# fakerlove1/HPFG

Hardware: AMD Instinct MI355X
Metric: labeled+unlabeled images/sec/node, U-Net 224x224 ACDC-shaped (Mean-Teacher step) (higher is better)
Workload: dtype bf16x3 (fp32 storage; products as split-bf16 MFMA hi*hi+hi*lo+lo*hi, fp32 accumulate); 1 GPU; mean_teacher_unet_224x224 (BASELINE configs[1]): U-Net 1ch->4cls, 8 labelled + 8 unlabelled per GPU, student fwd+bwd + train-mode teacher fwd + CE/Dice/MSE + SGD + EMA; size=224, hipgraph=True, sync_bn=False, parallelism=dp1, math=bf16x3

## Files before the change

### hpfg_amd/csrc/wgrad.hip

```cpp
#include <cstdlib>
#include "wgrad_kernel.h"
#include "wgrad_bf16_kernel.h"

namespace {

__global__ __launch_bounds__(256) void slab_reduce_kernel(const float* __restrict__ slab, float* __restrict__ dw, int S, int taps, int Cin,
                                                          int CinPad, int Cout, int CoutPad) {
  __shared__ float red[16][17];
  const long per = (long)taps * CinPad * CoutPad;
  const int il = threadIdx.x & 15, sl = threadIdx.x >> 4;
  const long i = (long)blockIdx.x * 16 + il;
  float t0 = 0.f, t1 = 0.f;
  if (i < per) {
    int s = sl;
    for (; s + 16 < S; s += 32) {
      t0 += slab[s * per + i];
      t1 += slab[(s + 16) * per + i];
    }
    if (s < S) t0 += slab[s * per + i];
  }
  red[sl][il] = t0 + t1;
  __syncthreads();
  if (sl == 0 && i < per) {
    float t = 0.f;
#pragma unroll
    for (int k = 0; k < 16; ++k) t += red[k][il];
    int co = (int)(i % CoutPad);
    int ci = (int)((i / CoutPad) % CinPad);
    int tap = (int)(i / ((long)CoutPad * CinPad));
    if (co < Cout && ci < Cin) dw[((long)co * Cin + ci) * taps + tap] = t;
  }
}

__global__ __launch_bounds__(256) void slab_reduce_multi_kernel(const HpfgSlabDesc* __restrict__ table) {
  __shared__ float red[16][65];
  const HpfgSlabDesc d = table[blockIdx.y];
  const long per = (long)d.taps * d.CinPad * d.CoutPad;
  const int il = threadIdx.x & 15, sl = threadIdx.x >> 4;
  const bool vec = (per & 3) == 0;
  for (long g0 = (long)blockIdx.x * 64; g0 < per; g0 += (long)gridDim.x * 64) {
    const long i = g0 + il * 4;
    f32x4 t0 = {0.f, 0.f, 0.f, 0.f}, t1 = t0;
    if (vec && i + 3 < per) {
      int s = sl;
      f32x4 t2 = t0, t3 = t0;
      for (; s + 48 < d.S; s += 64) {
        t0 += *reinterpret_cast<const f32x4*>(d.slab + s * per + i);
        t1 += *reinterpret_cast<const f32x4*>(d.slab + (s + 16) * per + i);
        t2 += *reinterpret_cast<const f32x4*>(d.slab + (s + 32) * per + i);
        t3 += *reinterpret_cast<const f32x4*>(d.slab + (s + 48) * per + i);
      }
      for (; s < d.S; s += 16) t0 += *reinterpret_cast<const f32x4*>(d.slab + s * per + i);
      t0 += t2;
      t1 += t3;
    } else {
      for (int s = sl; s < d.S; s += 16)
#pragma unroll
        for (int j = 0; j < 4; ++j)
          if (i + j < per) t0[j] += d.slab[s * per + i + j];
    }
    __syncthreads();
#pragma unroll
    for (int j = 0; j < 4; ++j) red[sl][il * 4 + j] = t0[j] + t1[j];
    __syncthreads();
    if (threadIdx.x < 64) {
      const long e = g0 + threadIdx.x;
      if (e < per) {
        float t = 0.f;
#pragma unroll
        for (int k = 0; k < 16; ++k) t += red[k][threadIdx.x];
        const int co = (int)(e % d.CoutPad), ci = (int)((e / d.CoutPad) % d.CinPad), tap = (int)(e / ((long)d.CoutPad * d.CinPad));
        if (co < d.Cout && ci < d.Cin) d.dw_oihw[((long)co * d.Cin + ci) * d.taps + tap] = t;
      }
    }
  }
}

__global__ __launch_bounds__(256) void channel_sum_stage1(const float* __restrict__ g, int pstride, long npix, int C, float* __restrict__ scratch) {
  __shared__ float red[256 * 4];
  const int tid = threadIdx.x;
  if ((C & 3) == 0 && (pstride & 3) == 0) {
    const int Q = C >> 2, q = tid % Q, pl = tid / Q, PL = 256 / Q;
    f32x4 a = {0.f, 0.f, 0.f, 0.f};
    if (pl < PL) {
      const long stride = (long)gridDim.x * PL;
      for (long pix = (long)blockIdx.x * PL + pl; pix < npix; pix += 4 * stride) {
#pragma unroll
        for (int u = 0; u < 4; ++u) {
          const long px = pix + u * stride;
          if (px < npix) a += *reinterpret_cast<const f32x4*>(g + px * pstride + q * 4);
        }
      }
    }
#pragma unroll
    for (int j = 0; j < 4; ++j) red[tid * 4 + j] = a[j];
    __syncthreads();
    if (tid < C) {
      float t = 0.f;
      const int qq = tid >> 2, j = tid & 3;
      for (int l = 0; l < PL; ++l) t += red[(l * Q + qq) * 4 + j];
      scratch[(long)blockIdx.x * C + tid] = t;
    }
    return;
  }
  const int c = tid % C, pl = tid / C, PL = 256 / C;
  float a = 0.f;
  if (pl < PL)
    for (long pix = (long)blockIdx.x * PL + pl; pix < npix; pix += (long)gridDim.x * PL) a += g[pix * pstride + c];
  red[tid] = a;
  __syncthreads();
  if (tid < C) {
    float t = 0.f;
    for (int l = 0; l < PL; ++l) t += red[l * C + tid];
    scratch[(long)blockIdx.x * C + tid] = t;
  }
}

__global__ __launch_bounds__(64) void channel_sum_stage2(const float* __restrict__ scratch, int nblk, int C, float* __restrict__ out) {
  const int c = blockIdx.x;
  double a = 0.0;
  for (int i = threadIdx.x; i < nblk; i += 64) a += (double)scratch[(long)i * C + c];
#pragma unroll
  for (int o = 32; o >= 1; o >>= 1) a += __shfl_xor(a, o);
  if (threadIdx.x == 0) out[c] = (float)a;
}

}

extern "C" int hpfg_wgrad_splits(int N, int H, int W, int CinPad, int CoutPad, int taps) {
  (void)taps;
  using namespace hpfg_wg;
  int ni, nj;
  hpfg_wg16::pick_shape(CinPad, CoutPad, &ni, &nj);
  long pairs = (long)(CinPad / (16 * ni)) * (CoutPad / (16 * nj));
  long nwork = (long)N * ((H + TH - 1) / TH) * ((W + TW - 1) / TW);
  const long resident = 512;
  long target = resident / pairs;
  if (target < 1) target = 1;
  if (target > nwork) target = nwork;
  long per_block = (nwork + target - 1) / target;
  return (int)((nwork + per_block - 1) / per_block);
}

extern "C" long hpfg_wgrad_slab_floats(int N, int H, int W, int CinPad, int CoutPad, int taps) {
  return (long)hpfg_wgrad_splits(N, H, W, CinPad, CoutPad, taps) * taps * CinPad * CoutPad;
}

extern "C" int hpfg_wgrad(const HpfgWgradArgs* a, void* stream) {
  HPFG_ARG_CHECK(a && a->slab && a->dw_oihw, "wgrad: null pointer");
  HPFG_ARG_CHECK(a->taps == 9 || a->taps == 1, "wgrad: taps must be 1 or 9");
  HPFG_ARG_CHECK(a->CinPad % 16 == 0 && a->CoutPad % 16 == 0 && a->Cin <= a->CinPad && a->Cout <= a->CoutPad, "wgrad: bad channel padding");
  HPFG_ARG_CHECK(a->S >= 1, "wgrad: S < 1");
  HPFG_ARG_CHECK(a->a1.mode == HPFG_ACT_NONE || a->a0.C % 16 == 0, "wgrad: concat needs a0.C %% 16 == 0");
  hipStream_t st = (hipStream_t)stream;
  const int akind = hpfg_kind_of(a->a0, a->a1);
  HPFG_ARG_CHECK(akind >= 0 && akind != HPFG_KIND_DZ, "wgrad: unsupported input source (a0.mode=%d, a1.mode=%d)", a->a0.mode, a->a1.mode);
  int rc = 1;
  const bool b16 = (a->math & 0xff) == HPFG_MATH_BF16X3 && a->taps == 9;
  if ((a->math & 0xff) == HPFG_MATH_BF16X3 && a->taps == 1 && (a->g.mode == HPFG_ACT_PLAIN || a->g.mode == HPFG_ACT_STRIDED) && a->g.C % 4 == 0)
    rc = hpfg_wgrad16_launch_1x1(*a, akind, st);
  if (a->g.mode == HPFG_ACT_SPLIT16 || akind == HPFG_KIND_SPLIT) {
    HPFG_ARG_CHECK(b16, "wgrad: SPLIT16 sources are a feature of the 3x3 bf16x3 kernel");
    rc = hpfg_wgrad16_launch_split(*a, akind, st);
  } else if (rc != 1) {
  } else if (b16 && a->g.mode == HPFG_ACT_DZ) rc = hpfg_wgrad16_launch_dz(*a, akind, st);
  else if (b16 && (a->g.mode == HPFG_ACT_PLAIN || a->g.mode == HPFG_ACT_STRIDED)) rc = hpfg_wgrad16_launch_plain(*a, akind, st);
  else if (a->g.mode == HPFG_ACT_DZ) rc = hpfg_wgrad_launch_dz(*a, akind, st);
  else if (a->g.mode == HPFG_ACT_PLAIN || a->g.mode == HPFG_ACT_STRIDED) rc = hpfg_wgrad_launch_plain(*a, akind, st);
  else {
    hpfg_set_error("wgrad: unsupported gradient source mode %d", a->g.mode);
    return -1;
  }
  if (rc || a->defer_reduce) return rc;
  long per = (long)a->taps * a->CinPad * a->CoutPad;
  hipLaunchKernelGGL(slab_reduce_kernel, dim3((unsigned)((per + 15) / 16)), dim3(256), 0, st, a->slab, a->dw_oihw, a->S, a->taps, a->Cin, a->CinPad,
                     a->Cout, a->CoutPad);
  return hpfg_launch_status("slab_reduce_kernel");
}

extern "C" int hpfg_slab_reduce_multi(const HpfgSlabDesc* table_dev, const HpfgSlabDesc* table_host, int nlayers, void* stream) {
  HPFG_ARG_CHECK(table_dev && table_host && nlayers > 0 && nlayers < 65536, "slab_reduce_multi: bad args");
  long mx = 0;
  for (int i = 0; i < nlayers; ++i) {
    long per = (long)table_host[i].taps * table_host[i].CinPad * table_host[i].CoutPad;
    if (per > mx) mx = per;
  }
  long gx = (mx + 63) / 64;
  if (gx > 2048) gx = 2048;
  hipLaunchKernelGGL(slab_reduce_multi_kernel, dim3((unsigned)gx, nlayers), dim3(256), 0, (hipStream_t)stream, table_dev);
  return hpfg_launch_status("slab_reduce_multi_kernel");
}

extern "C" int hpfg_channel_sum_blocks(long npix, int C) {
  if (C < 1 || C > 256 || npix < 1) return 0;
  const int PL = 256 / C;
  const long want = (npix + PL - 1) / PL;
  return (int)(want < 512 ? want : 512);
}

extern "C" int hpfg_channel_sum_partials(const float* g, int pstride, long npix, int C, float* partials, void* stream) {
  HPFG_ARG_CHECK(g && partials && C >= 1 && C <= 256 && npix > 0, "channel_sum_partials: bad args");
  hipLaunchKernelGGL(channel_sum_stage1, dim3(hpfg_channel_sum_blocks(npix, C)), dim3(256), 0, (hipStream_t)stream, g, pstride, npix, C, partials);
  return hpfg_launch_status("channel_sum_stage1");
}

extern "C" int hpfg_channel_sum(const float* g, int pstride, long npix, int C, float* out, float* scratch, void* stream) {
  HPFG_ARG_CHECK(g && out && scratch && C >= 1 && C <= 256 && npix > 0, "channel_sum: bad args");
  int PL = 256 / C;
  long want = (npix + PL - 1) / PL;
  int nblk = (int)(want < 512 ? want : 512);
  hipLaunchKernelGGL(channel_sum_stage1, dim3(nblk), dim3(256), 0, (hipStream_t)stream, g, pstride, npix, C, scratch);
  hipLaunchKernelGGL(channel_sum_stage2, dim3(C), dim3(64), 0, (hipStream_t)stream, scratch, nblk, C, out);
  return hpfg_launch_status("channel_sum");
}
```

Baseline: 7877 images/s.

## Rewrite multi-layer slab reduction with per-layer geometry plans and flattened grid

Replaces the 2D-grid slab reduction, where every layer got the same number of blocks sized by the largest layer, with a flattened 1D grid. A host-computed plan gives each layer exactly the blocks it needs. Each layer picks one of four strategies from its shape: a few-slab quad path that transposes through LDS for coalesced OIHW writes, lane and part paths with deep batched loads for many slabs, or a scalar row fallback. The aim is to remove idle blocks, increase memory-level parallelism and improve write coalescing, at the cost of much more complex code and a per-block linear search for its layer.

```diff
diff --git a/hpfg_amd/csrc/wgrad.hip b/hpfg_amd/csrc/wgrad.hip
--- a/hpfg_amd/csrc/wgrad.hip
+++ b/hpfg_amd/csrc/wgrad.hip
@@ -32,47 +32,269 @@
   }
 }
 
-__global__ __launch_bounds__(256) void slab_reduce_multi_kernel(const HpfgSlabDesc* __restrict__ table) {
-  __shared__ float red[16][65];
-  const HpfgSlabDesc d = table[blockIdx.y];
+constexpr int SR_THREADS = 256;
+constexpr int SR_MAX_LAYERS = 32;
+constexpr int SR_LDS_FLOATS = 1152;
+enum { SR_QUAD = 0, SR_LANES = 1, SR_PARTS = 2, SR_ROWS = 3 };
+
+struct SrGeom {
+  int kind, CW, R, ncb, nrb;
+};
+struct SrPlan {
+  int n;
+  int start[SR_MAX_LAYERS + 1];
+};
+
+__host__ __device__ HPFG_NO_PK_F32 inline SrGeom sr_geom(const HpfgSlabDesc& d) {
+  SrGeom g;
   const long per = (long)d.taps * d.CinPad * d.CoutPad;
-  const int il = threadIdx.x & 15, sl = threadIdx.x >> 4;
-  const bool vec = (per & 3) == 0;
-  for (long g0 = (long)blockIdx.x * 64; g0 < per; g0 += (long)gridDim.x * 64) {
-    const long i = g0 + il * 4;
-    f32x4 t0 = {0.f, 0.f, 0.f, 0.f}, t1 = t0;
-    if (vec && i + 3 < per) {
-      int s = sl;
-      f32x4 t2 = t0, t3 = t0;
-      for (; s + 48 < d.S; s += 64) {
-        t0 += *reinterpret_cast<const f32x4*>(d.slab + s * per + i);
-        t1 += *reinterpret_cast<const f32x4*>(d.slab + (s + 16) * per + i);
-        t2 += *reinterpret_cast<const f32x4*>(d.slab + (s + 32) * per + i);
-        t3 += *reinterpret_cast<const f32x4*>(d.slab + (s + 48) * per + i);
+  g.CW = g.R = 0, g.nrb = 1;
+  if (d.CinPad % 16 || d.CoutPad % 16 || ((uintptr_t)d.slab & 15)) {
+    g.kind = SR_ROWS, g.ncb = (int)((per + 15) / 16);
+  } else if (d.S <= 16) {
+    g.kind = SR_QUAD;
+    g.CW = d.CoutPad % 32 == 0 ? 32 : 16;
+    g.R = SR_THREADS / (d.taps * (g.CW / 4));
+    g.ncb = (d.Cout + g.CW - 1) / g.CW;
+    g.nrb = (d.Cin + g.R - 1) / g.R;
+  } else {
+    const int nq = d.taps * d.Cin * ((d.Cout + 3) / 4);
+    g.kind = d.S > 256 && per < (1L << 23) ? SR_PARTS : SR_LANES;
+    g.ncb = g.kind == SR_PARTS ? (nq + 3) / 4 : (nq + 15) / 16;
+  }
+  return g;
+}
+
+__device__ __forceinline__ HPFG_NO_PK_F32 void sr_barrier() {
+  __builtin_amdgcn_fence(__ATOMIC_RELEASE, "workgroup");
+  __builtin_amdgcn_s_barrier();
+  __builtin_amdgcn_fence(__ATOMIC_ACQUIRE, "workgroup");
+}
+
+#define SR_GLOBAL __attribute__((address_space(1)))
+template <typename T>
+__device__ __forceinline__ HPFG_NO_PK_F32 T sr_ld(const float* row, unsigned vbyte) {
+  return *(const SR_GLOBAL T*)((const SR_GLOBAL char*)row + vbyte);
+}
+
+template <typename T, int B>
+__device__ __forceinline__ HPFG_NO_PK_F32 void sr_batch(const float*& row, long rs, unsigned vbyte, T& t0, T& t1, T& t2, T& t3) {
+  T x[B];
+#pragma unroll
+  for (int i = 0; i < B; ++i) x[i] = sr_ld<T>(row + i * rs, vbyte);
+#pragma unroll
+  for (int i = 0; i < B; i += 4) {
+    t0 += x[i];
+    t1 += x[i + 1];
+    t2 += x[i + 2];
+    t3 += x[i + 3];
+  }
+  row += B * rs;
+}
+
+template <typename T>
+__device__ __forceinline__ HPFG_NO_PK_F32 T sr_chain(const float* row, long rs, unsigned vbyte, int nfull, bool extra) {
+  T t0{}, t1{}, t2{}, t3{};
+  int n4 = nfull & ~3;
+  const int rem = nfull & 3;
+  for (; n4 >= 16; n4 -= 16) sr_batch<T, 16>(row, rs, vbyte, t0, t1, t2, t3);
+  if (n4 >= 8) {
+    sr_batch<T, 8>(row, rs, vbyte, t0, t1, t2, t3);
+    n4 -= 8;
+  }
+  if (n4 >= 4) sr_batch<T, 4>(row, rs, vbyte, t0, t1, t2, t3);
+  T x0{}, x1{}, x2{}, xe{};
+  if (rem > 0) x0 = sr_ld<T>(row, vbyte);
+  if (rem > 1) x1 = sr_ld<T>(row + rs, vbyte);
+  if (rem > 2) x2 = sr_ld<T>(row + 2 * rs, vbyte);
+  if (extra) xe = sr_ld<T>(row + rem * rs, vbyte);
+  if (rem == 3) {
+    t0 += x0;
+    t1 = extra ? t1 + x1 : t1;
+    t0 = extra ? t0 : t0 + x1;
+    t2 = extra ? t2 + x2 : t2;
+    t0 = extra ? t0 : t0 + x2;
+    t3 = extra ? t3 + xe : t3;
+  } else {
+    if (rem > 0) t0 += x0;
+    if (rem > 1) t0 += x1;
+    t0 = extra ? t0 + xe : t0;
+  }
+  t0 += t2;
+  t1 += t3;
+  return t0 + t1;
+}
+
+template <int NR>
+__device__ __forceinline__ HPFG_NO_PK_F32 f32x4 sr_chain_once(const float* row, long rs, unsigned vbyte, int nfull, bool extra) {
+  f32x4 x[NR], xe{};
+#pragma unroll
+  for (int i = 0; i < NR; ++i) x[i] = sr_ld<f32x4>(row + (i < nfull ? i : nfull - 1) * rs, vbyte);
+  if (extra) xe = sr_ld<f32x4>(row + nfull * rs, vbyte);
+  const int g4 = nfull & ~3;
+  const bool grp = (nfull & 3) == 3 && extra;
+  f32x4 t[4] = {};
+#pragma unroll
+  for (int i = 0; i < NR; ++i) {
+    if (i < g4) {
+      t[i & 3] += x[i];
+    } else if (i < nfull) {
+      if ((i & 3) == 0) {
+        t[0] += x[i];
+      } else {
+        t[i & 3] = grp ? t[i & 3] + x[i] : t[i & 3];
+        t[0] = grp ? t[0] : t[0] + x[i];
       }
-      for (; s < d.S; s += 16) t0 += *reinterpret_cast<const f32x4*>(d.slab + s * per + i);
-      t0 += t2;
-      t1 += t3;
-    } else {
-      for (int s = sl; s < d.S; s += 16)
-#pragma unroll
-        for (int j = 0; j < 4; ++j)
-          if (i + j < per) t0[j] += d.slab[s * per + i + j];
-    }
-    __syncthreads();
-#pragma unroll
-    for (int j = 0; j < 4; ++j) red[sl][il * 4 + j] = t0[j] + t1[j];
-    __syncthreads();
-    if (threadIdx.x < 64) {
-      const long e = g0 + threadIdx.x;
-      if (e < per) {
-        float t = 0.f;
-#pragma unroll
-        for (int k = 0; k < 16; ++k) t += red[k][threadIdx.x];
-        const int co = (int)(e % d.CoutPad), ci = (int)((e / d.CoutPad) % d.CinPad), tap = (int)(e / ((long)d.CoutPad * d.CinPad));
-        if (co < d.Cout && ci < d.Cin) d.dw_oihw[((long)co * d.Cin + ci) * d.taps + tap] = t;
+    }
+  }
+  t[3] = grp ? t[3] + xe : t[3];
+  t[0] = extra && !grp ? t[0] + xe : t[0];
+  t[0] += t[2];
+  t[1] += t[3];
+  return t[0] + t[1];
+}
+
+template <int B>
+__device__ __forceinline__ HPFG_NO_PK_F32 void sr_serial(const float* row, long rs, unsigned vbyte, int n, f32x4& t) {
+  f32x4 x[B];
+#pragma unroll
+  for (int i = 0; i < B; ++i) x[i] = sr_ld<f32x4>(row + (i < n ? i : n - 1) * rs, vbyte);
+#pragma unroll
+  for (int i = 0; i < B; ++i)
+    if (i < n) t += x[i];
+}
+
+__device__ __forceinline__ HPFG_NO_PK_F32 f32x4 sr_part(const float* slab, long per, unsigned vbyte, int p, int S) {
+  const int nfull = S >> 4, rem = nfull & 3, a = p >> 4;
+  const bool extra = (p & 15) < (S & 15);
+  const bool grp = rem == 3 && extra;
+  const int m = rem + (extra ? 1 : 0);
+  const long rs = 64 * per;
+  int n = nfull >> 2;
+  const float* tail = slab + n * rs;
+  f32x4 y0{}, y1{}, y2{};
+  const bool l0 = grp || (a == 0 && m > 0), l1 = !grp && a == 0 && m > 1, l2 = !grp && a == 0 && m > 2;
+  if (l0) y0 = sr_ld<f32x4>(tail, vbyte);
+  if (l1) y1 = sr_ld<f32x4>(tail + 16 * per, vbyte);
+  if (l2) y2 = sr_ld<f32x4>(tail + 32 * per, vbyte);
+  f32x4 t{};
+  const float* row = slab;
+  for (; n > 16; n -= 16) {
+    f32x4 x[16];
+#pragma unroll
+    for (int i = 0; i < 16; ++i) x[i] = sr_ld<f32x4>(row + i * rs, vbyte);
+#pragma unroll
+    for (int i = 0; i < 16; ++i) t += x[i];
+    row += 16 * rs;
+  }
+  if (n > 8) sr_serial<16>(row, rs, vbyte, n, t);
+  else if (n > 0) sr_serial<8>(row, rs, vbyte, n, t);
+  t = l0 ? t + y0 : t;
+  t = l1 ? t + y1 : t;
+  t = l2 ? t + y2 : t;
+  return t;
+}
+
+template <int NR>
+__device__ __forceinline__ HPFG_NO_PK_F32 f32x4 sr_few(const float* row, long per, unsigned vbyte, int S) {
+  f32x4 x[NR];
+#pragma unroll
+  for (int k = 0; k < NR; ++k) x[k] = sr_ld<f32x4>(row + (k < S ? k : S - 1) * per, vbyte);
+  f32x4 t{};
+  const f32x4 zero{};
+#pragma unroll
+  for (int k = 0; k < NR; ++k) {
+    f32x4 t0 = zero, t1 = zero;
+    t0 += x[k];
+    t0 += zero;
+    t1 += zero;
+    const f32x4 red = t0 + t1;
+    if (k < S) t += red;
+  }
+  return t;
+}
+
+__global__ __launch_bounds__(SR_THREADS) HPFG_NO_PK_F32 void slab_reduce_multi_kernel(const HpfgSlabDesc* __restrict__ table, const SrPlan plan) {
+  __shared__ __attribute__((aligned(16))) float lds[SR_LDS_FLOATS];
+  int layer = 0;
+  while (layer + 1 < plan.n && (int)blockIdx.x >= plan.start[layer + 1]) ++layer;
+  const HpfgSlabDesc d = table[layer];
+  const SrGeom g = sr_geom(d);
+  const int item = (int)blockIdx.x - plan.start[layer];
+  const long per = (long)d.taps * d.CinPad * d.CoutPad;
+  const int tid = threadIdx.x;
+  SR_GLOBAL float* dw = (SR_GLOBAL float*)d.dw_oihw;
+  if (g.kind == SR_ROWS) {
+    const int sl = tid >> 4, el = tid & 15;
+    const long e = (long)item * 16 + el;
+    const int co = (int)(e % d.CoutPad), ci = (int)((e / d.CoutPad) % d.CinPad), tap = (int)(e / ((long)d.CoutPad * d.CinPad));
+    const bool real = e < per && co < d.Cout && ci < d.Cin;
+    lds[tid] = real ? sr_chain<float>(d.slab, 16 * per, (unsigned)(sl * per + e) * 4u, d.S >> 4, sl < (d.S & 15)) : 0.f;
+    sr_barrier();
+    if (sl == 0 && real) {
+      float t = 0.f;
+#pragma unroll
+      for (int k = 0; k < 16; ++k) t += lds[k * 16 + el];
+      dw[((long)co * d.Cin + ci) * d.taps + tap] = t;
+    }
+    return;
+  }
+  if (g.kind != SR_QUAD) {
+    const int cqa = (d.Cout + 3) >> 2, nq = d.taps * d.Cin * cqa;
+    const int sh = g.kind == SR_LANES ? 4 : 2, nql = 1 << sh;
+    const int p = tid >> sh, q = item * nql + (tid & (nql - 1));
+    f32x4 v{};
+    if (q < nq) {
+      const int row = q / cqa, cq = q - row * cqa, tap = row / d.Cin, ci = row - tap * d.Cin;
+      const unsigned vb = (unsigned)(p * per + (tap * d.CinPad + ci) * d.CoutPad + cq * 4) * 4u;
+      const int nfull = d.S >> 4;
+      const bool extra = p < (d.S & 15);
+      if (g.kind == SR_PARTS) v = sr_part(d.slab, per, vb, p, d.S);
+      else if (nfull <= 2) v = sr_chain_once<2>(d.slab, 16 * per, vb, nfull, extra);
+      else if (nfull <= 4) v = sr_chain_once<4>(d.slab, 16 * per, vb, nfull, extra);
+      else if (nfull <= 8) v = sr_chain_once<8>(d.slab, 16 * per, vb, nfull, extra);
+      else if (nfull <= 16) v = sr_chain_once<16>(d.slab, 16 * per, vb, nfull, extra);
+      else v = sr_chain<f32x4>(d.slab, 16 * per, vb, nfull, extra);
+    }
+    *reinterpret_cast<f32x4*>(lds + tid * 4) = v;
+    sr_barrier();
+    const int ne = nql * 4, q2 = item * nql + (tid >> 2);
+    if (tid < ne && q2 < nq) {
+      const int row = q2 / cqa, cq = q2 - row * cqa, tap = row / d.Cin, ci = row - tap * d.Cin, co = cq * 4 + (tid & 3);
+      float t = 0.f;
+      if (g.kind == SR_PARTS) {
+#pragma unroll
+        for (int k = 0; k < 16; ++k) {
+          const float t0 = lds[k * ne + tid] + lds[(k + 32) * ne + tid], t1 = lds[(k + 16) * ne + tid] + lds[(k + 48) * ne + tid];
+          t += t0 + t1;
+        }
+      } else {
+#pragma unroll
+        for (int k = 0; k < 16; ++k) t += lds[k * ne + tid];
       }
-    }
+      if (co < d.Cout) dw[((long)co * d.Cin + ci) * d.taps + tap] = t;
+    }
+    return;
+  }
+  const int cb = item % g.ncb, rb = item / g.ncb;
+  const int co0 = cb * g.CW, ci0 = rb * g.R;
+  const int ract = d.Cin - ci0 < g.R ? d.Cin - ci0 : g.R;
+  const int cow = d.Cout - co0 < g.CW ? d.Cout - co0 : g.CW;
+  const int cqa = (cow + 3) >> 2, w1 = cqa * 4 + 1;
+  const int nrow = d.taps * ract, nq = nrow * cqa;
+  const float* base = d.slab + (long)ci0 * d.CoutPad + co0;
+  for (int q = tid; q < nq; q += SR_THREADS) {
+    const int row = q / cqa, cq = q - row * cqa, tap = row / ract, r = row - tap * ract;
+    const unsigned vb = (unsigned)((tap * d.CinPad + r) * d.CoutPad + cq * 4) * 4u;
+    const f32x4 t = d.S <= 8 ? sr_few<8>(base, per, vb, d.S) : sr_few<16>(base, per, vb, d.S);
+#pragma unroll
+    for (int j = 0; j < 4; ++j) lds[row * w1 + cq * 4 + j] = t[j];
+  }
+  sr_barrier();
+  const int per_co = ract * d.taps;
+  for (int o = tid; o < cow * per_co; o += SR_THREADS) {
+    const int c = o / per_co, rt = o - c * per_co, r = rt / d.taps, tap = rt - r * d.taps;
+    dw[((long)(co0 + c) * d.Cin + ci0) * d.taps + rt] = lds[(tap * ract + r) * w1 + c];
   }
 }
 
@@ -180,14 +402,29 @@
 
 extern "C" int hpfg_slab_reduce_multi(const HpfgSlabDesc* table_dev, const HpfgSlabDesc* table_host, int nlayers, void* stream) {
   HPFG_ARG_CHECK(table_dev && table_host && nlayers > 0 && nlayers < 65536, "slab_reduce_multi: bad args");
-  long mx = 0;
   for (int i = 0; i < nlayers; ++i) {
-    long per = (long)table_host[i].taps * table_host[i].CinPad * table_host[i].CoutPad;
-    if (per > mx) mx = per;
-  }
-  long gx = (mx + 63) / 64;
-  if (gx > 2048) gx = 2048;
-  hipLaunchKernelGGL(slab_reduce_multi_kernel, dim3((unsigned)gx, nlayers), dim3(256), 0, (hipStream_t)stream, table_dev);
+    const HpfgSlabDesc& d = table_host[i];
+    HPFG_ARG_CHECK(d.slab && d.dw_oihw && d.S >= 1, "slab_reduce_multi: layer %d: null pointer or S < 1", i);
+    HPFG_ARG_CHECK(d.taps == 9 || d.taps == 1, "slab_reduce_multi: layer %d: taps must be 1 or 9", i);
+    HPFG_ARG_CHECK(d.Cin >= 1 && d.Cin <= d.CinPad && d.Cout >= 1 && d.Cout <= d.CoutPad, "slab_reduce_multi: layer %d: bad channel padding", i);
+    HPFG_ARG_CHECK((d.CinPad % 16 == 0 && d.CoutPad % 16 == 0) || (d.taps == 1 && d.CinPad == 1),
+                   "slab_reduce_multi: layer %d: paddings %d x %d are neither multiples of 16 nor a row table", i, d.CinPad, d.CoutPad);
+    HPFG_ARG_CHECK((long)d.taps * d.CinPad * d.CoutPad < (1L << 26), "slab_reduce_multi: layer %d: too large", i);
+  }
+  for (int l0 = 0; l0 < nlayers; l0 += SR_MAX_LAYERS) {
+    SrPlan plan;
+    plan.n = nlayers - l0 < SR_MAX_LAYERS ? nlayers - l0 : SR_MAX_LAYERS;
+    long at = 0;
+    for (int i = 0; i <= SR_MAX_LAYERS; ++i) {
+      plan.start[i] = (int)at;
+      if (i < plan.n) {
+        const SrGeom g = sr_geom(table_host[l0 + i]);
+        at += (long)g.ncb * g.nrb;
+      }
+    }
+    HPFG_ARG_CHECK(at < (1L << 30), "slab_reduce_multi: too many work items");
+    hipLaunchKernelGGL(slab_reduce_multi_kernel, dim3((unsigned)at), dim3(SR_THREADS), 0, (hipStream_t)stream, table_dev + l0, plan);
+  }
   return hpfg_launch_status("slab_reduce_multi_kernel");
 }
 
```

After: 7890 images/s, median of 4. About the same (+0.2%).
